# ace19-dev/gvcnn-tf

Hardware: AMD Instinct MI355X
Metric: views/sec (higher is better)
Workload: dtype f32; 1 GPU; BASELINE.json configs[1]: ModelNet-shaped, 12 views x 224x224x3, inception_v3 backbone (raw tap Mixed_6e, final tap Mixed_7c), num_groups=7, f32, forward only; views_per_gpu=384, global_views=384, num_groups=7, num_classes=10, exchange=none, branch_lanes=3, launch=eager

## Files before the change

gvcnn-tf_amd/backbones.py:

```python
import ctypes as C
import os

import numpy as np
import torch

from . import _lib

INCEPTION_BN_EPS = 0.001
RESNET_BN_EPS = 1e-5

INCEPTION_ENDPOINTS = [
    "Conv2d_1a_3x3", "Conv2d_2a_3x3", "Conv2d_2b_3x3", "MaxPool_3a_3x3", "Conv2d_3b_1x1",
    "Conv2d_4a_3x3", "MaxPool_5a_3x3", "Mixed_5b", "Mixed_5c", "Mixed_5d", "Mixed_6a", "Mixed_6b",
    "Mixed_6c", "Mixed_6d", "Mixed_6e", "Mixed_7a", "Mixed_7b", "Mixed_7c"]

SLOT_INPUT, SLOT_WEIGHTS, SLOT_SS, SLOT_ACT0 = 0, 1, 2, 3


def _same_pads(in_size, k, s):
    out = -(-in_size // s)
    total = max((out - 1) * s + k - in_size, 0)
    return out, total // 2


# ... 554 lines not shown
            if kind in ("bias", "bias_sum"):
                for n in name.split("|"):
                    shapes[n] = (c,)
            else:
                for leaf in ("beta", "moving_mean", "moving_variance") + (("gamma",) if has_gamma else ()):
                    shapes[name + "/" + leaf] = (c,)
        return shapes

    def _ptr_table(self, x):
        assert x.is_contiguous() and x.dtype == torch.float32
        assert x.numel() == self.nb * self.height * self.width * 3, (tuple(x.shape), self.nb)
        if self._ptrs is None:
            self._ptrs = (C.c_void_p * len(self._bufs))()
            for i, b in enumerate(self._bufs):
                self._ptrs[i] = b.data_ptr() if b is not None else 0
        self._ptrs[SLOT_INPUT] = x.data_ptr()
        return self._ptrs

    def run(self, x, stream=None):
        ptrs = self._ptr_table(x)
        _lib.check(self.lib.gv_plan_run(self._plan, ptrs, len(self._bufs), _stream_ptr(stream)),
                   "gv_plan_run")

    def run_range(self, x, first, count, stream=None):
        ptrs = self._ptr_table(x)
        _lib.check(self.lib.gv_plan_run_range(self._plan, first, count, ptrs, len(self._bufs),
                                              _stream_ptr(stream)), "gv_plan_run_range")

    def declined_fused_pools(self):
        fused = [i for i, op in enumerate(self.ops) if op["kind"] == "conv" and (op.get("maxpool") or op.get("chain"))]
        if not fused:
            return []
        x = torch.zeros(self.nb * self.height * self.width * 3, dtype=torch.float32, device=self.weights.device)
        declined = []
        for i in fused:
            rc = self.lib.gv_plan_run_range(self._plan, i, 1, self._ptr_table(x), len(self._bufs), _stream_ptr(None))
            if rc == _lib.GV_E_UNSUPPORTED:
                declined.append(self.ops[i]["name"])
            else:
                _lib.check(rc, "gv_plan_run_range(%s)" % self.ops[i]["name"])
        torch.cuda.synchronize(self.weights.device)
        self._ptrs[SLOT_INPUT] = 0
        return declined

    def apply_tiles(self, table):
        for i, op in enumerate(self.ops):
            if op["kind"] == "conv" and op["name"] in table and not op.get("maxpool") and not op.get("chain"):
                op["tile"] = int(table[op["name"]]) + 1
                _lib.check(self.lib.gv_plan_set_conv_tile(self._plan, i, op["tile"]), "gv_plan_set_conv_tile")

    def autotune(self, x, iters=3, verbose=False, in_sequence=4):
        lib = self.lib
        ncfg_plan = lib.gv_conv2d_num_tile_cfgs(self.math_mode if self.dtype == _lib.GV_F32 else -1)
        ncfg_p3 = lib.gv_conv2d_num_tile_cfgs(-3)
        self.run(x)
        chosen, cands = {}, {}
        try:
            for i, op in enumerate(self.ops):
                if op["kind"] != "conv" or op.get("chain"):
                    continue
                ncfg = ncfg_p3 if op["x"].p3 else ncfg_plan
                timed = []
                for t in range(ncfg):
                    lib.gv_conv2d_set_tile_override(t)
                    try:
                        timed.append((self.time_range(x, i, 1, iters), t))
                    except _lib.GvError:
                        continue
                finals = []
                for _, t in sorted(timed)[:3]:
                    lib.gv_conv2d_set_tile_override(t)
                    finals.append((min(self.time_range(x, i, 1, 2 * iters), self.time_range(x, i, 1, 2 * iters)), t))
                best_ms, best = min(finals) if finals else (float("inf"), 0)
                op["tile"] = best + 1
                chosen[op["name"]] = (best, best_ms)
                order = [best] + [t for _, t in sorted(timed) if t != best]
                cands[i] = order[:max(int(in_sequence), 1)]
                _lib.check(lib.gv_plan_set_conv_tile(self._plan, i, best + 1), "gv_plan_set_conv_tile")
                if verbose:
                    print("autotune %-60s cfg %2d  %.4f ms" % (op["name"][-60:], best, best_ms))
        finally:
            lib.gv_conv2d_set_tile_override(-1)
        if int(in_sequence) > 1 and cands:
            seq = {i: {} for i in cands}
            for r in range(int(in_sequence)):
                for i, c in cands.items():
                    _lib.check(lib.gv_plan_set_conv_tile(self._plan, i, c[min(r, len(c) - 1)] + 1), "gv_plan_set_conv_tile")
                each = [min(a, b) for a, b in zip(self.time_each(x, 2 * iters), self.time_each(x, 2 * iters))]
                for i, c in cands.items():
                    t = c[min(r, len(c) - 1)]
                    seq[i][t] = min(each[i], seq[i].get(t, float("inf")))
            moved = 0
            for i, c in cands.items():
                op = self.ops[i]
                best = min(c, key=lambda t: (seq[i][t], c.index(t)))
                moved += best != c[0]
                op["tile"] = best + 1
                chosen[op["name"]] = (best, seq[i][best])
                _lib.check(lib.gv_plan_set_conv_tile(self._plan, i, best + 1), "gv_plan_set_conv_tile")
                if verbose:
                    print("in sequence %-57s cfg %2d  %.4f ms  (warm-repeat choice cfg %2d: %.4f ms in sequence)"
                          % (op["name"][-57:], best, seq[i][best], c[0], seq[i][c[0]]))
            self.autotune_moved = moved
        return chosen

    def time_range(self, x, first, count, iters, stream=None):
# ... 351 lines not shown
```

gvcnn-tf_amd/csrc/conv_bf16s.hip:

```cpp
#include <type_traits>

#include "conv_common.h"
#include "conv_x3_epi.h"

namespace {

using gvconv::ConvArgs;

typedef __bf16 bf16x8 __attribute__((ext_vector_type(8)));
typedef __bf16 bf16x2 __attribute__((ext_vector_type(2)));
typedef unsigned u32x4 __attribute__((ext_vector_type(4)));

constexpr int KT = 16;

__host__ __device__ constexpr int prod_count(int np) { return np == 3 ? 6 : (np == 2 ? 3 : 1); }
__host__ __device__ constexpr int prod_pa(int np, int t) {
    return np == 3 ? (t == 0 ? 2 : (t == 2 || t == 3 ? 1 : 0)) : (np == 2 ? (t == 0 ? 1 : 0) : 0);
}
__host__ __device__ constexpr int prod_pb(int np, int t) {
    return np == 3 ? (t == 1 ? 2 : (t == 2 || t == 4 ? 1 : 0)) : (np == 2 ? (t == 1 ? 1 : 0) : 0);
}

template <int NP>
__device__ __forceinline__ void split8(f32x4 lo, f32x4 hi, bool ok, u32x4 (&out)[NP]) {
// ... 1138 lines not shown
template <int WM, int WN, int TM, int TN, int NP>
int launch_cfg(const ConvArgs& a0, bool generic, hipStream_t st) {
    constexpr int BM = WM * TM * 32, BN = WN * TN * 32;
    ConvArgs a = a0;
    a.tiles_n = gv_ceil_div(a.cout, BN);
    const int tiles_m = gv_ceil_div(a.M, BM);
    const int64_t nwg = (int64_t)tiles_m * a.tiles_n;
    if (nwg > 0x7fffffff) return GV_E_UNSUPPORTED;
    size_t lds = (size_t)(2 * BM + 2 * BN) * (NP * 32 + 16) + (generic ? (size_t)a.Kpad * 8 : 0);
    if (a.y_p3 | a.y2_p3) {
        const size_t epi = (size_t)(WM * WN) * X3EpiGeom<TN>::BYTES;
        lds = lds > epi ? lds : epi;
    }
    if (generic) {
        if (lds > 64 * 1024) {
            const bool ok = GV_BIG_LDS_OK((&conv_igemm_bf16s<WM, WN, TM, TN, NP, true>), 160 * 1024);
            if (!ok) return GV_E_UNSUPPORTED;
        }
        hipLaunchKernelGGL((conv_igemm_bf16s<WM, WN, TM, TN, NP, true>), dim3((unsigned)nwg), dim3(WM * WN * 64), lds, st, a);
    } else {
        if (lds > 64 * 1024) {
            const bool ok = GV_BIG_LDS_OK((&conv_igemm_bf16s<WM, WN, TM, TN, NP, false>), 160 * 1024);
            if (!ok) return GV_E_UNSUPPORTED;
        }
        hipLaunchKernelGGL((conv_igemm_bf16s<WM, WN, TM, TN, NP, false>), dim3((unsigned)nwg), dim3(WM * WN * 64), lds, st, a);
    }
    GV_LAUNCH_CHECK();
    return GV_OK;
}

template <int NP>
int launch_np(int cfg, const ConvArgs& a, bool generic, hipStream_t st) {
    switch (cfg) {
        case 0: return launch_cfg<2, 2, 2, 2, NP>(a, generic, st);
        case 1: return launch_cfg<2, 2, 2, 1, NP>(a, generic, st);
        case 2: return launch_cfg<2, 2, 1, 1, NP>(a, generic, st);
        case 3: return launch_cfg<4, 1, 1, 3, NP>(a, generic, st);
        case 4: return launch_cfg<2, 2, 1, 2, NP>(a, generic, st);
        case 5: return launch_cfg<4, 1, 1, 1, NP>(a, generic, st);
        case 6: return launch_cfg<4, 2, 2, 2, NP>(a, generic, st);
        case 7: return launch_cfg<2, 4, 2, 2, NP>(a, generic, st);
        case 8: return launch_cfg<4, 2, 2, 1, NP>(a, generic, st);
        case 9: return launch_cfg<2, 2, 2, 3, NP>(a, generic, st);
        case 10: return launch_cfg<2, 2, 1, 3, NP>(a, generic, st);
    }
    return GV_E_UNSUPPORTED;
}

}

namespace gvconv {

int bf16s_num_cfgs() { return kNumTiles + 1 + wsg_x3_num_cfgs(); }
int bf16s_special_cfg() { return kNumTiles; }

bool bf16s_stem_ok(int planes, const ConvArgs& a) {
    return planes == 3 && !a.y_p3 && a.cin == 3 && a.kh == a.kw && (a.kw == 3 || a.kw == 7) && a.stride == 2 && a.cout <= 64 &&
           a.dil_shift == 0 && a.split == 0 && a.y2 == nullptr && a.res == nullptr &&
           (int64_t)a.nb * a.ih * a.iw * a.x_ld < 0x7fffffffll;
}

bool bf16s_halo_ok(int planes, const ConvArgs& a, bool generic) {
    return planes == 3 && !generic && !a.y_p3 && a.kh == 3 && a.kw == 3 && a.stride == 1 && a.cin == 32 && a.cout <= 64 &&
           a.dil_shift == 0 && a.split == 0 && a.y2 == nullptr && a.oh == a.ih + 2 * a.pad_t - 2 &&
           a.ow == a.iw + 2 * a.pad_l - 2;
}

bool bf16s_halo_pool_ok(int planes, const ConvArgs& a, bool generic) {
    return a.pool == 1 && bf16s_halo_ok(planes, a, generic) && a.res == nullptr && a.cout % 4 == 0 && a.oh >= 3 && a.ow >= 3 &&
           !(gv_ceil_div(a.ow, 16) * 16 * 5 <= gv_ceil_div(a.ow, 30) * 32 * 4);
}

int bf16s_pick_tile(int , int M, int N, int ) {
    int best = 0;
    double best_cost = 1e30;
    const int order[] = {0, 3, 1, 5};
    const double pen[] = {1.00, 1.02, 1.05, 1.20};
    for (int t = 0; t < 4; ++t) {
        const int bn = kTiles[order[t]].bn;
        const double cost = (double)gv_ceil_div(N, bn) * bn * pen[t];
        if (cost < best_cost) { best_cost = cost; best = order[t]; }
    }
    const int64_t blocks = (int64_t)gv_ceil_div(M, 128) * gv_ceil_div(N, kTiles[best].bn);
    if (blocks < 1024) {
        if (kTiles[best].bn == 128) best = 4;
        else if (kTiles[best].bn == 64) best = 2;
    }
    return best;
}

int bf16s_launch(int planes, int cfg, const ConvArgs& a0, bool generic, hipStream_t st) {
    ConvArgs a = a0;
    a.Kpad = (a.K + KT - 1) / KT * KT;
    a.ktiles = a.Kpad / KT;
    if (cfg == kNumTiles) {
        if (a.pool) return bf16s_halo_pool_ok(planes, a, generic) ? launch_halo_x3(a, st) : GV_E_UNSUPPORTED;
        if (bf16s_stem_ok(planes, a)) return launch_stem_x3(a, st);
        return bf16s_halo_ok(planes, a, generic) ? launch_halo_x3(a, st) : GV_E_UNSUPPORTED;
    }
    if (cfg > kNumTiles) return planes == 3 && !generic ? wsg_x3_launch(cfg - kNumTiles - 1, a0, st) : GV_E_UNSUPPORTED;
    switch (planes) {
        case 3: return launch_np<3>(cfg, a, generic, st);
        case 2: return launch_np<2>(cfg, a, generic, st);
        case 1: return launch_np<1>(cfg, a, generic, st);
    }
    return GV_E_UNSUPPORTED;
// ... 25 lines not shown
```

gvcnn-tf_amd/csrc/conv_common.h:

```cpp
#pragma once
#include "gv_common.h"
#include "conv_stats.h"

namespace gvconv {

struct ConvArgs {
    const float* x;
    const void* w;
    const float* scale;
    const float* shift;
    const float* res;
    float* y;
    float* y2;
    const float* scale2;
    const float* shift2;
    int nb, ih, iw, cin, x_ld;
    int kh, kw, stride, pad_t, pad_l;
    int oh, ow, cout, y_ld, res_ld, y2_ld;
    int M, K, Kpad, ktiles;
    int relu, relu2, split;
    int relu_limit;
    int tiles_n;
    int dil_shift;
#ifdef GV_PHASE_TIMES
// ... 59 lines not shown
                const int m = rbase + (r & 3) + 8 * (r >> 2);
                if (m >= a.M) continue;
                float v = acc[i][j][r] * sc + sh;
                if (a.res) v += a.res[(size_t)m * a.res_ld + col];
                if (dual) {
                    float v2 = v * sc2 + sh2;
                    if (a.relu2) v2 = fmaxf(v2, 0.f);
                    a.y2[(size_t)m * a.y2_ld + col] = v2;
                }
                if (relu) v = fmaxf(v, 0.f);
                ybase[(size_t)m * yld] = v;
            }
        }
    }
}

int bf16s_num_cfgs();
int bf16s_special_cfg();
int bf16s_pick_tile(int planes, int M, int N, int K);
bool bf16s_halo_ok(int planes, const ConvArgs& a, bool generic);
bool bf16s_halo_pool_ok(int planes, const ConvArgs& a, bool generic);
bool bf16s_stem_ok(int planes, const ConvArgs& a);
int bf16s_launch(int planes, int cfg, const ConvArgs& a, bool generic, hipStream_t st);
int bf16s_pack_filter(const float* w_hwio, int kh, int kw, int cin, int cout, int planes, void* out,
                      hipStream_t st);
int64_t bf16s_packed_bytes(int kh, int kw, int cin, int cout, int planes);


int lp_num_cfgs();
int lp_pick_tile(int M, int N, int K);
bool lp_xpre_cfg_ok(int cfg);
int lp_xpre_pick(int M, int N);
bool lp_halo_ok(const ConvArgs& a, bool generic);
bool lp_halo_pool_ok(const ConvArgs& a, bool generic);
bool lp_stem_pool_ok(const ConvArgs& a, bool xf32);
bool lp_stem_ok(const ConvArgs& a, bool xf32);
int lp_launch(int dtype, int cfg, const ConvArgs& a, bool generic, bool xf32, hipStream_t st);
int lp_pack_filter(const float* w_hwio, int kh, int kw, int cin, int cout, int dtype, void* out, hipStream_t st);
int64_t lp_packed_bytes(int kh, int kw, int cin, int cout);
int lp_pack_filters_batched(const gv_pack_job* jobs_dev, const int* block_job_dev, int nblocks, int dtype, hipStream_t st);
int lp_special_cfg();

int dma_lp_num_cfgs();
bool dma_lp_ok(const ConvArgs& a, bool generic, bool xf32);
int dma_lp_launch(int dtype, int cfg, const ConvArgs& a, hipStream_t st);
const void* dma_zero_page();
bool chain_tail_ok(const ConvArgs& a);
int chain_tail_launch(int dtype, const ConvArgs& a, hipStream_t st);
int ws_lp_num_cfgs();
int ws_lp_launch(int dtype, int cfg, const ConvArgs& a, hipStream_t st);
int dma_x3_num_cfgs();
bool dma_x3_ok(const ConvArgs& a);
int dma_x3_launch(int cfg, const ConvArgs& a, hipStream_t st);
int ws_x3_num_cfgs();
int ws_x3_launch(int cfg, const ConvArgs& a, hipStream_t st);
int wsg_x3_num_cfgs();
int wsg_x3_launch(int cfg, const ConvArgs& a, hipStream_t st);

}
```

gvcnn-tf_amd/csrc/conv_igemm.hip:

```cpp
#include "conv_common.h"

namespace {

using gvconv::ConvArgs;

constexpr int CH = 16;
constexpr int KPAD_ALIGN = 32;

template <int WM, int WN, int TM, int TN, int NCH, bool GENERIC>
__global__ __launch_bounds__(256) void conv_igemm_f32(const ConvArgs a) {
    static_assert(WM * WN == 4, "4 waves per workgroup");
    constexpr int BM = WM * TM * 32;
    constexpr int BN = WN * TN * 32;
    constexpr int BKT = CH * NCH;
    constexpr int LDS_LD = BKT + 4;
    constexpr int QPR = BKT / 4;
    constexpr int A_LOADS = (BM * QPR + 255) / 256;
    constexpr int B_LOADS = (BN * QPR + 255) / 256;

    extern __shared__ __attribute__((aligned(16))) float smem[];
    float* sA = smem;
    float* sB = smem + 2 * BM * LDS_LD;

    const int tid = threadIdx.x;
// ... 258 lines not shown
        case 9: return launch_cfg<4, 1, 1, 1, 2>(a, generic, st);
        case 10: return launch_cfg<2, 2, 1, 1, 2>(a, generic, st);
        case 11: return launch_cfg<2, 2, 1, 2, 2>(a, generic, st);
    }
    return GV_E_UNSUPPORTED;
}

int pick_tile(int M, int N, int K) {
    int best = 1;
    double best_cost = 1e30;
    const int order[] = {0, 2, 1, 3};
    const double pen[] = {1.00, 1.00, 1.03, 1.10};
    for (int t = 0; t < 4; ++t) {
        const int bn = kTiles[order[t]].bn;
        const double cost = (double)gv_ceil_div(N, bn) * bn * pen[t];
        if (cost < best_cost) { best_cost = cost; best = order[t]; }
    }
    const int64_t blocks = (int64_t)gv_ceil_div(M, 128) * gv_ceil_div(N, kTiles[best].bn);
    if (blocks < 1024) {
        if (kTiles[best].bn == 128) best = 5;
        else if (kTiles[best].bn == 64) best = 4;
    }
    if (K >= 64) best += 6;
    return best;
}

}

extern "C" void gv_conv2d_set_tile_override(int cfg) { g_tile_override = cfg; }
extern "C" void gv_conv2d_set_debug(int bits) { g_debug = bits; }
#ifdef GV_PHASE_TIMES
unsigned long long* g_phase_buf = nullptr;
extern "C" void gv_conv2d_set_phase_buffer(void* p) { g_phase_buf = (unsigned long long*)p; }
#endif
static int planes_of(int math_mode) {
    switch (math_mode) {
        case GV_MATH_F32: return 0;
        case GV_MATH_BF16X3: return 3;
        case GV_MATH_BF16X2: return 2;
        case GV_MATH_BF16X1: return 1;
    }
    return -1;
}

extern "C" int gv_conv2d_special_tile_cfg(int32_t math_mode) {
    if (math_mode == -1) return gvconv::lp_special_cfg();
    const int np = planes_of(math_mode);
    return np <= 0 ? GV_E_BADARG : gvconv::bf16s_special_cfg();
}

extern "C" int gv_conv2d_num_tile_cfgs(int32_t math_mode) {
    if (math_mode == -1) return gvconv::lp_num_cfgs();
    if (math_mode == -3) return gvconv::dma_x3_num_cfgs();
    const int np = planes_of(math_mode);
    return np < 0 ? GV_E_BADARG : (np == 0 ? kNumTiles : gvconv::bf16s_num_cfgs());
}

extern "C" int64_t gv_packed_filter_bytes(int32_t kh, int32_t kw, int32_t cin, int32_t cout,
                                          int32_t dtype, int32_t math_mode) {
    if (kh <= 0 || kw <= 0 || cin <= 0 || cout <= 0) return GV_E_BADARG;
    if (dtype == GV_BF16 || dtype == GV_F16) return gvconv::lp_packed_bytes(kh, kw, cin, cout);
    if (dtype != GV_F32) return GV_E_UNSUPPORTED;
    const int np = planes_of(math_mode);
    if (np < 0) return GV_E_BADARG;
    if (np > 0) return gvconv::bf16s_packed_bytes(kh, kw, cin, cout, np);
    const int64_t K = (int64_t)kh * kw * cin;
    return 4 * (int64_t)cout * ((K + KPAD_ALIGN - 1) / KPAD_ALIGN * KPAD_ALIGN);
}

extern "C" int gv_pack_filter_hwio(const float* w_hwio, int32_t kh, int32_t kw, int32_t cin,
                                   int32_t cout, void* w_packed, int32_t dtype, int32_t math_mode,
                                   void* stream) {
    if (!w_hwio || !w_packed || kh <= 0 || kw <= 0 || cin <= 0 || cout <= 0) return GV_E_BADARG;
    if (dtype == GV_BF16 || dtype == GV_F16)
        return gvconv::lp_pack_filter(w_hwio, kh, kw, cin, cout, dtype, w_packed, (hipStream_t)stream);
    if (dtype != GV_F32) return GV_E_UNSUPPORTED;
    const int np = planes_of(math_mode);
    if (np < 0) return GV_E_BADARG;
    if (np > 0) return gvconv::bf16s_pack_filter(w_hwio, kh, kw, cin, cout, np, w_packed, (hipStream_t)stream);
    const int K = kh * kw * cin;
    const int Kpad = (K + KPAD_ALIGN - 1) / KPAD_ALIGN * KPAD_ALIGN;
    const int64_t total = (int64_t)cout * Kpad;
    hipLaunchKernelGGL(pack_filter_hwio_f32, dim3((unsigned)gv_ceil_div(total, 256)), dim3(256), 0,
                       (hipStream_t)stream, w_hwio, K, Kpad, cout, (float*)w_packed);
    GV_LAUNCH_CHECK();
    return GV_OK;
}

extern "C" int gv_pack_filters_batched(const gv_pack_job* jobs_dev, int32_t num_jobs, const int32_t* block_job_dev,
                                       int32_t num_blocks, int32_t dtype, void* stream) {
    if (!jobs_dev || !block_job_dev || num_jobs <= 0 || num_blocks <= 0) return GV_E_BADARG;
    if (dtype != GV_BF16 && dtype != GV_F16) return GV_E_UNSUPPORTED;
    return gvconv::lp_pack_filters_batched(jobs_dev, block_job_dev, num_blocks, dtype, (hipStream_t)stream);
}

static int conv2d_fwd_impl(const gv_conv_desc* d, const void* x, const float* xscale, const float* xshift,
                           const void* w_packed, const float* scale, const float* shift, const void* residual,
                           void* y, void* y2, const float* scale2, const float* shift2, void* stream,
                           const gv_bn_stats* stats = nullptr);

extern "C" int gv_conv2d_fwd(const gv_conv_desc* d, const void* x, const void* w_packed,
                             const float* scale, const float* shift, const void* residual,
                             void* y, void* y2, const float* scale2, const float* shift2,
                             void* stream) {
    return conv2d_fwd_impl(d, x, nullptr, nullptr, w_packed, scale, shift, residual, y, y2, scale2, shift2, stream);
}
// ... 4 lines not shown
                                  const float* shift2, void* stream) {
    if (!xscale || !xshift) return GV_E_BADARG;
    return conv2d_fwd_impl(d, x, xscale, xshift, w_packed, scale, shift, residual, y, y2, scale2, shift2, stream);
}

extern "C" int gv_conv2d_fwd_bnstats(const gv_conv_desc* d, const void* x, const void* w_packed, const float* scale,
                                     const float* shift, const void* residual, void* y, const gv_bn_stats* stats,
                                     void* stream) {
    if (!stats) return GV_E_BADARG;
    return conv2d_fwd_impl(d, x, nullptr, nullptr, w_packed, scale, shift, residual, y, nullptr, nullptr, nullptr, stream, stats);
}

static int conv2d_fwd_impl(const gv_conv_desc* d, const void* x, const float* xscale, const float* xshift,
                           const void* w_packed, const float* scale, const float* shift, const void* residual,
                           void* y, void* y2, const float* scale2, const float* shift2, void* stream,
                           const gv_bn_stats* stats) {
    if (!d || !x || !w_packed || !scale || !shift || !y) return GV_E_BADARG;
    if (d->nb <= 0 || d->ih <= 0 || d->iw <= 0 || d->cin <= 0 || d->cout <= 0 || d->kh <= 0 ||
        d->kw <= 0 || d->stride <= 0 || d->oh <= 0 || d->ow <= 0 || d->pad_t < 0 || d->pad_l < 0)
        return GV_E_BADARG;
    const bool split = (d->flags & GV_CONV_SPLIT) != 0;
    if (split) {
        if (!y2 || d->split_col <= 0 || d->split_col >= d->cout) return GV_E_BADARG;
        if (d->y_ld < d->split_col || d->y2_ld < d->cout - d->split_col) return GV_E_BADARG;
    } else {
        if (d->y_ld < d->cout) return GV_E_BADARG;
        if (y2 && (!scale2 || !shift2 || d->y2_ld < d->cout)) return GV_E_BADARG;
    }
    if (d->x_ld < d->cin) return GV_E_BADARG;
    if (residual && d->res_ld < d->cout) return GV_E_BADARG;
    {
        if (d->in_dilation != 2 && d->y_step != 2 && ((d->oh - 1) * d->stride - d->pad_t >= d->ih ||
                                    (d->ow - 1) * d->stride - d->pad_l >= d->iw))
            return GV_E_BADARG;
    }
    const bool lp = d->dtype == GV_BF16 || d->dtype == GV_F16;
    if (d->dtype != GV_F32 && !lp) return GV_E_UNSUPPORTED;
    if ((d->flags & GV_CONV_X_F32) && !lp) return GV_E_BADARG;
    const int np = lp ? 1 : planes_of(d->math_mode);
    if (np < 0) return GV_E_BADARG;
    const bool xp3 = (d->flags & GV_CONV_X_P3) != 0;
    const bool yp3 = (d->flags & GV_CONV_Y_P3) != 0, y2p3 = (d->flags & GV_CONV_Y2_P3) != 0;
    if ((xp3 || yp3 || y2p3) && (lp || np != 3)) return GV_E_BADARG;
    if (y2p3 && !split) return GV_E_BADARG;
    if (yp3 || y2p3) {
        if (d->cout % 8 != 0 || (y2 && !split) || (residual && d->res_ld % 4 != 0)) return GV_E_UNSUPPORTED;
        if (yp3 && (d->y_ld % 16 != 0 || (split ? d->split_col : d->cout) % 16 != 0)) return GV_E_UNSUPPORTED;
        if (y2p3 && (d->y2_ld % 16 != 0 || (d->cout - d->split_col) % 16 != 0 || d->split_col % 8 != 0)) return GV_E_UNSUPPORTED;
        if (!yp3 && (d->y_ld % 4 != 0 || !gv_aligned16(y))) return GV_E_ALIGN;
        if (split && !y2p3 && (d->y2_ld % 4 != 0 || !gv_aligned16(y2))) return GV_E_ALIGN;
        if (split && d->split_col % 8 != 0) return GV_E_UNSUPPORTED;
    }
    const int ncfg = lp ? gvconv::lp_num_cfgs()
                        : (xp3 ? gvconv::dma_x3_num_cfgs() : (np == 0 ? kNumTiles : gvconv::bf16s_num_cfgs()));
    if (d->tile_cfg < 0 || d->tile_cfg > ncfg) return GV_E_BADARG;
    const int64_t M64 = (int64_t)d->nb * d->oh * d->ow;
    if (M64 > 0x7fffffff || (int64_t)d->nb * d->ih * d->iw > 0x7fffffff) return GV_E_UNSUPPORTED;
    if (!gv_aligned16(w_packed)) return GV_E_ALIGN;

    ConvArgs a;
    a.x = (const float*)x; a.w = w_packed; a.scale = scale; a.shift = shift;
    a.res = (const float*)residual; a.y = (float*)y; a.y2 = (float*)y2;
    a.scale2 = scale2; a.shift2 = shift2;
    a.xscale = xscale; a.xshift = xshift;
    a.nb = d->nb; a.ih = d->ih; a.iw = d->iw; a.cin = d->cin; a.x_ld = d->x_ld;
    a.kh = d->kh; a.kw = d->kw; a.stride = d->stride; a.pad_t = d->pad_t; a.pad_l = d->pad_l;
    a.oh = d->oh; a.ow = d->ow; a.cout = d->cout; a.y_ld = d->y_ld; a.res_ld = d->res_ld;
    a.y2_ld = d->y2_ld;
    a.M = (int)M64; a.K = d->kh * d->kw * d->cin;
    a.Kpad = (a.K + KPAD_ALIGN - 1) / KPAD_ALIGN * KPAD_ALIGN;
    a.ktiles = 0;
    a.relu = (d->flags & GV_CONV_RELU) ? 1 : 0;
    a.relu2 = (d->flags & GV_CONV_RELU2) ? 1 : 0;
    a.split = split ? d->split_col : 0;
    if (d->relu_cols < 0) return GV_E_BADARG;
    a.relu_limit = d->relu_cols > 0 ? d->relu_cols : 0x7fffffff;
    a.tiles_n = 0;
    a.dbg = g_debug;
#ifdef GV_PHASE_TIMES
    a.phase_buf = g_phase_buf;
#endif
    a.zeros = nullptr;
    a.y_p3 = (d->flags & GV_CONV_Y_P3) ? 1 : 0;
    a.y2_p3 = (d->flags & GV_CONV_Y2_P3) ? 1 : 0;
    if (d->in_dilation != 0 && d->in_dilation != 1 && d->in_dilation != 2) return GV_E_BADARG;
    a.dil_shift = d->in_dilation == 2 ? 1 : 0;
    if (a.dil_shift && (np == 0 || (d->cin % CH != 0) || d->stride != 1)) return GV_E_UNSUPPORTED;
    if (d->y_step != 0) {
        if (d->y_step != 2 || d->y_py < 0 || d->y_py > 1 || d->y_px < 0 || d->y_px > 1) return GV_E_BADARG;
        if (2 * (d->oh - 1) + d->y_py >= d->y_ih || 2 * (d->ow - 1) + d->y_px >= d->y_iw) return GV_E_BADARG;
        if (!lp || split || y2 || d->stride != 1 || a.dil_shift) return GV_E_UNSUPPORTED;
        if ((int64_t)d->nb * d->y_ih * d->y_iw > 0x7fffffff) return GV_E_UNSUPPORTED;
        a.y_step = 2; a.y_py = d->y_py; a.y_px = d->y_px; a.y_ih = d->y_ih; a.y_iw = d->y_iw;
    }
    a.y_div_img = gv_fast_div(d->oh * d->ow);
    a.y_div_row = gv_fast_div(d->ow);
    if (stats) {
        if (stats->mode != GV_BN_STATS_FWD && stats->mode != GV_BN_STATS_BWD) return GV_E_BADARG;
        if (stats->groups <= 0 || stats->nseg <= 0 || stats->nseg > GV_BN_STATS_MAX_SEG) return GV_E_BADARG;
        if (!lp || split || y2 || (d->flags & (GV_CONV_RELU | GV_CONV_RELU2))) return GV_E_UNSUPPORTED;
        if (d->cout % 8 != 0 || d->y_ld % 8 != 0 || !gv_aligned16(y) || (residual && (d->res_ld % 8 != 0 || !gv_aligned16(residual))))
            return GV_E_UNSUPPORTED;
        a.st.mode = stats->mode == GV_BN_STATS_FWD ? gvconv::STAT_FWD : gvconv::STAT_BWD;
        a.st.hw = d->oh * d->ow;
        a.st.G = stats->groups;
        a.st.nseg = stats->nseg;
        a.st.hw_magic = a.st.hw > 1 ? (unsigned)((0x100000000ull + (unsigned)a.st.hw - 1) / (unsigned)a.st.hw) : 0u;
// ... 111 lines not shown
```

gvcnn-tf_amd/csrc/conv_ws_x3.hip:

```cpp
#include <cstdlib>
#include <type_traits>

#include "conv_common.h"
#include "conv_lp_epi.h"
#include "conv_x3_epi.h"

namespace {

constexpr int X3W_HEAD = 64;
constexpr int X3W_NL = 4;

struct WsX3Args {
    int taps, nchunks, nk;
    int halo_lo;
    int strip_blocks;
    int pad_[3];
};

__device__ __forceinline__ void x3w_dma16(const char* gsrc, char* lds_dst) {
    __builtin_amdgcn_global_load_lds((const __attribute__((address_space(1))) void*)gsrc,
                                     (__attribute__((address_space(3))) void*)lds_dst, 16, 0, 0);
}
template <int N>
__device__ __forceinline__ void x3w_wait_vm() {
    static_assert(N >= 0 && N < 64, "vmcnt is a 6-bit counter");
    asm volatile("s_waitcnt vmcnt(%0)" ::"n"(N) : "memory");
}

__device__ __forceinline__ void x3w_gload16(f32x4& dst, const char* p) {
    asm volatile("global_load_dwordx4 %0, %1, off" : "=v"(dst) : "v"(p) : "memory");
}
template <int N>
__device__ __forceinline__ void x3w_wait_vm_reg(f32x4& r) {
    static_assert(N >= 0 && N < 64, "vmcnt is a 6-bit counter");
    asm volatile("s_waitcnt vmcnt(%1)" : "+v"(r) : "n"(N) : "memory");
}

template <int WM, int WN, int TM, int TN, int NB, int SBMAX, int GEMM = 0>
__global__ __launch_bounds__((WM * WN + X3W_NL) * 64, 3) void conv_ws_x3(const ConvArgs a, const WsX3Args w) {
    constexpr int NC = WM * WN;
    constexpr int BM = WM * TM * 32, BN = WN * TN * 32;
    constexpr int B_PLANE = BN * 32, B_SLOT = 3 * B_PLANE;
    constexpr int A_PLANE = GEMM ? BM * 32 : X3W_HEAD + SBMAX * 1024, S_BUF = 3 * A_PLANE;
    constexpr int NA = GEMM ? 3 : 2;
    constexpr int OFF_S = NB * B_SLOT;
    constexpr int UB3 = 3 * (BN / 32);
    constexpr int LB = (UB3 + X3W_NL - 1) / X3W_NL;
    static_assert(NC == 8, "eight consumer waves + four loaders: three waves per SIMD");
    static_assert(TM <= TN && TM * TN >= 4, "plane-2 fragments of a and b share one register block");
    static_assert(NB >= 3 && (NB - 1) * LB < 64, "ring depth / vmcnt range");
    static_assert(GEMM == 0 || (NB == 4 && BM % (16 * X3W_NL) == 0), "GEMM mode: four filter slots, 16-row load instructions");
    (void)NA;

    extern __shared__ __attribute__((aligned(128))) char smem[];
    const int tid = threadIdx.x;
    const int lane = tid & 63;
    const int wave = __builtin_amdgcn_readfirstlane(tid >> 6);
    const int lid = gv_xcd_remap(blockIdx.x, gridDim.x);
    const int tile_n = lid % a.tiles_n, tile_m = lid / a.tiles_n;
    const int m0 = tile_m * BM, n0 = tile_n * BN;
    const int nk = w.nk, NTAP = w.taps;
    const bool nosync = (a.dbg & (16384 | 65536)) != 0;

    static_assert(BN <= X3W_NL * 64, "one loader thread per tile column");
    float ss_v[2] = {0.f, 0.f};
    f32x16 acc[TM][TN];

    if (wave >= NC) {
        const int lw = wave - NC;
        if (tid - NC * 64 < BN) {
            const int cc = min(n0 + tid - NC * 64, a.cout - 1);
            ss_v[0] = a.scale[cc];
            ss_v[1] = a.shift[cc];
        }
        if (!(a.dbg & 16384)) {
            __builtin_amdgcn_s_setprio(3);
            const bool nodma = (a.dbg & 32768) != 0, nobar = (a.dbg & 65536) != 0;
            const int lrow = lane >> 1;
            const int lc16 = (((lane & 1) ^ ((lrow >> 3) & 1)) << 4);
            const char* xb = reinterpret_cast<const char*>(a.x);
            const char* b_ptr[LB];
            int b_dst[LB];
            {
                const size_t wrow = (size_t)(a.Kpad / 16) * 96;
#pragma unroll
                for (int i = 0; i < LB; ++i) {
                    int d = lw + i * X3W_NL;
                    d = d < UB3 ? d : UB3 - 1;
                    const int rb = d / 3, p = d - rb * 3;
                    int n = n0 + rb * 32 + lrow;
                    n = n < a.cout ? n : a.cout - 1;
                    b_ptr[i] = reinterpret_cast<const char*>(a.w) + (size_t)n * wrow + p * 32 + lc16;
                    b_dst[i] = p * B_PLANE + rb * 1024;
                }
            }
            int bq_t = 0, bq_c = 0, bq_slot = 0;
            const int gtap = (a.cin >> 4) * 96;
            auto issue_b = [&]() {
                const unsigned koff = (unsigned)(bq_t * gtap + bq_c * 96);
                char* sb = smem + bq_slot * B_SLOT;
#pragma unroll
                for (int i = 0; i < LB; ++i)
                    if (!nodma) x3w_dma16(b_ptr[i] + koff, sb + b_dst[i]);
                if (++bq_t == NTAP) { bq_t = 0; ++bq_c; }
                bq_slot = bq_slot + 1 == NB ? 0 : bq_slot + 1;
            };
            if constexpr (GEMM != 0) {
                constexpr int RPW = BM / X3W_NL, NI = RPW / 16;
                const int qd = lane & 3;
                const char* a_ptr[NI];
                int a_dst[NI];
#pragma unroll
                for (int i = 0; i < NI; ++i) {
                    const int row = lw * RPW + i * 16 + (lane >> 2);
                    int m = m0 + row;
                    m = m < a.M ? m : a.M - 1;
                    a_ptr[i] = xb + (size_t)(unsigned)m * ((size_t)a.x_ld * 4) + qd * 16;
                    a_dst[i] = OFF_S + row * 32 + ((((qd >> 1) ^ ((row >> 3) & 1))) << 4) + (qd & 1) * 8;
                }
                f32x4 stg[2][NI];
                auto load_a = [&](auto sc, int c) {
                    constexpr int S = decltype(sc)::value;
                    c = c < nk ? c : nk - 1;
#pragma unroll
                    for (int i = 0; i < NI; ++i) x3w_gload16(stg[S][i], a_ptr[i] + (size_t)c * 64);
                };
                auto wait_a = [&](auto sc, auto nc) {
                    constexpr int S = decltype(sc)::value;
                    constexpr int N = decltype(nc)::value;
#pragma unroll
                    for (int i = 0; i < NI; ++i) x3w_wait_vm_reg<N>(stg[S][i]);
                };
                auto write_a = [&](auto sc, int slot) {
                    constexpr int S = decltype(sc)::value;
                    char* sb = smem + slot * S_BUF;
#pragma unroll
                    for (int i = 0; i < NI; ++i) {
                        float v[4] = {stg[S][i][0], stg[S][i][1], stg[S][i][2], stg[S][i][3]};
#pragma unroll
                        for (int p = 0; p < 3; ++p) {
                            const unsigned lo = pack2<__bf16>(v[0], v[1]), hi = pack2<__bf16>(v[2], v[3]);
                            typedef unsigned u32x2_t __attribute__((ext_vector_type(2)));
                            *reinterpret_cast<u32x2_t*>(sb + p * A_PLANE + a_dst[i]) = u32x2_t{lo, hi};
                            if (p < 2) {
                                v[0] -= __builtin_bit_cast(float, lo << 16);
                                v[1] -= __builtin_bit_cast(float, lo & 0xffff0000u);
                                v[2] -= __builtin_bit_cast(float, hi << 16);
                                v[3] -= __builtin_bit_cast(float, hi & 0xffff0000u);
                            }
                        }
                    }
                };
                using S0 = std::integral_constant<int, 0>;
                using S1 = std::integral_constant<int, 1>;
                auto fetch = [&](auto sc, int k) {
                    issue_b();
                    load_a(sc, k);
                };
                fetch(S0{}, 0);
                fetch(S1{}, 1);
                wait_a(S0{}, std::integral_constant<int, 0>{});
                wait_a(S1{}, std::integral_constant<int, 0>{});
                write_a(S0{}, 0);
                write_a(S1{}, 1);
                fetch(S0{}, 2);
                fetch(S1{}, 3);
                asm volatile("s_waitcnt lgkmcnt(0)" ::: "memory");
                if (!nobar) __builtin_amdgcn_s_barrier();
                auto iter = [&](auto sc, int j) {
                    wait_a(sc, std::integral_constant<int, LB + NI>{});
                    if (j + 2 < nk) {
                        int slot = j + 2;
                        slot -= (slot / 3) * 3;
                        write_a(sc, slot);
                        asm volatile("s_waitcnt lgkmcnt(0)" ::: "memory");
                    }
                    if (!nobar) __builtin_amdgcn_s_barrier();
                    if (j + 4 >= nk) {
                        bq_c = nk - 1;
                        bq_slot = (nk - 1) & 3;
                    }
                    fetch(sc, j + 4);
                };
                for (int j = 0; j + 1 < nk; j += 2) {
                    iter(S0{}, j);
                    if (j + 2 < nk) iter(S1{}, j + 1);
                }
                x3w_wait_vm<0>();
            } else {
            const unsigned pix_bytes = (unsigned)a.x_ld * 6u;
            int sq_c = 0, sq_buf = 0;
            int sp_blk = 1 << 30, sp_p = 0, sp_c = 0, sp_buf = 0;
            auto strip_begin = [&]() {
                sp_blk = lw / 3; sp_p = lw - sp_blk * 3; sp_c = sq_c; sp_buf = sq_buf;
                ++sq_c;
                sq_buf ^= 1;
            };
            auto strip_units = [&](int n) {
                char* sb = smem + OFF_S + sp_buf * S_BUF + X3W_HEAD;
                const unsigned coff = (unsigned)sp_c * 96u + (unsigned)lc16;
                for (int i = 0; i < n && sp_blk < w.strip_blocks; ++i) {
                    int p = m0 - w.halo_lo + sp_blk * 32 + lrow;
                    p = p < 0 ? 0 : (p < a.M ? p : a.M - 1);
                    if (!nodma) x3w_dma16(xb + (size_t)(unsigned)p * pix_bytes + coff + sp_p * 32, sb + sp_p * A_PLANE + sp_blk * 1024);
                    ++sp_p; ++sp_blk;
                    if (sp_p == 3) { sp_p = 0; ++sp_blk; }
                }
            };
            const int upl = (3 * w.strip_blocks + X3W_NL - 1) / X3W_NL;
            const int win = max(NTAP - NB + 2, 1);
            const int ppi = (upl + win - 1) / win;
            strip_begin();
            strip_units(1 << 20);
            issue_b();
#pragma unroll
            for (int q = 1; q < NB; ++q) issue_b();
            x3w_wait_vm<(NB - 2) * LB>();
            if (!nobar) __builtin_amdgcn_s_barrier();
            if (w.nchunks > 1) { strip_begin(); strip_units(ppi); }
            int ft = 0;
            for (int j = 0; j + 1 < nk; ++j) {
                if (j + NB - 1 <= nk - 1) x3w_wait_vm<(NB - 3) * LB>();
                else x3w_wait_vm<0>();
                if (!nobar) __builtin_amdgcn_s_barrier();
                const bool last_tap = ft + 1 == NTAP;
                if (last_tap && sq_c < w.nchunks) strip_begin();
                strip_units(ppi);
                if (j + NB < nk) issue_b();
                ft = last_tap ? 0 : ft + 1;
            }
            x3w_wait_vm<0>();
            }
        }
    } else {
        const int wm = wave / WN, wn = wave % WN;
        const int r = lane & 31, h = lane >> 5;
        if constexpr (GEMM == 0) {
            if (tid < 96) {
                const int img = tid >> 4;
// ... 102 lines not shown
                    if (j == TN - 1) { A1[i] = lds16(aa[i] + A_PLANE); X3W_PIN(); }
                    if (i == TM - 1) { B1[j] = lds16(bn + j * 1024 + B_PLANE); X3W_PIN(); }
                }
            }
            X3W_PIN();
        };
        int q_fr = 0, q_fs = 0, q_tap = 0;
        int sbuf = 0, bslot = 0;
        int aa[TM];
#pragma unroll
        for (int i = 0; i < TM; ++i) aa[i] = a_addr(i, -(a.pad_t * a.iw + a.pad_l), 0, OFF_S);
        asm volatile("s_waitcnt lgkmcnt(0)" ::: "memory");
        if (!nosync) __builtin_amdgcn_s_barrier();
#pragma unroll
        for (int i = 0; i < TM; ++i) { A0[i] = lds16(aa[i]); A1[i] = lds16(aa[i] + A_PLANE); }
#pragma unroll
        for (int j = 0; j < TN; ++j) {
            B0[j] = lds16(b_lane + j * 1024);
            B1[j] = lds16(b_lane + j * 1024 + B_PLANE);
            T[j] = lds16(b_lane + j * 1024 + 2 * B_PLANE);
        }
        int bn = 0;
        auto next_addr = [&]() {
            if constexpr (GEMM != 0) {
                sbuf = sbuf + 1 == NA ? 0 : sbuf + 1;
#pragma unroll
                for (int i = 0; i < TM; ++i) aa[i] = a_addr(i, 0, 0, OFF_S + sbuf * S_BUF);
                bslot = bslot + B_SLOT == NB * B_SLOT ? 0 : bslot + B_SLOT;
                bn = b_lane + bslot;
                return;
            }
            const bool wrap = q_tap + 1 == NTAP;
            const bool row_end = q_fs + 1 == a.kw;
            q_tap = wrap ? 0 : q_tap + 1;
            q_fr = wrap ? 0 : (row_end ? q_fr + 1 : q_fr);
            q_fs = (wrap || row_end) ? 0 : q_fs + 1;
            sbuf = wrap ? sbuf ^ 1 : sbuf;
            const int sbase = OFF_S + sbuf * S_BUF;
            const int off = (q_fr - a.pad_t) * a.iw + (q_fs - a.pad_l);
#pragma unroll
            for (int i = 0; i < TM; ++i) aa[i] = a_addr(i, off, q_tap, sbase);
            bslot = bslot + B_SLOT == NB * B_SLOT ? 0 : bslot + B_SLOT;
            bn = b_lane + bslot;
        };
        for (int j = 0; j + 1 < nk; ++j) {
            kstep(std::true_type{}, aa, bn, !nosync, next_addr);
        }
        kstep(std::false_type{}, aa, bn, false, [] {});
#undef X3W_PIN
    }
    __syncthreads();
    constexpr int SS_OFF = NC * X3EpiGeom<TN>::BYTES;
    float* sstab = reinterpret_cast<float*>(smem + SS_OFF);
    if (tid >= NC * 64 && tid - NC * 64 < BN) {
        sstab[tid - NC * 64] = ss_v[0];
        sstab[BN + tid - NC * 64] = ss_v[1];
    }
    __syncthreads();
    if (wave < NC) {
        const int wm = wave / WN, wn = wave % WN;
        x3_epilogue_staged<TM, TN>(a, acc, m0, n0, wm, wn, lane, reinterpret_cast<float*>(smem + wave * X3EpiGeom<TN>::BYTES), sstab, BN);
    }
}

#ifndef GV_KERNEL_ONLY
bool ws_x3_epi_ok(const ConvArgs& a) {
    if (a.cout % 8 != 0 || (a.y2 != nullptr && a.split == 0)) return false;
    if (a.res != nullptr && (a.res_ld % 4 != 0 || !gv_aligned16(a.res))) return false;
    if (!a.y_p3 && (a.y_ld % 4 != 0 || !gv_aligned16(a.y))) return false;
    if (a.split > 0 && (a.split % 8 != 0 || (!a.y2_p3 && (a.y2_ld % 4 != 0 || !gv_aligned16(a.y2))))) return false;
    return true;
}

bool ws_x3_shape_ok(const ConvArgs& a) {
    return a.stride == 1 && a.dil_shift == 0 && a.oh == a.ih && a.ow == a.iw && a.cin % 16 == 0 && a.x_ld % 16 == 0 &&
           a.kh * a.kw <= 32 && a.kw < 32 && a.pad_t < a.kh && a.pad_l < a.kw && a.pool == 0 && a.xscale == nullptr &&
           a.y_step == 0 && a.st.mode == gvconv::STAT_OFF && ws_x3_epi_ok(a);
}

template <int WM, int WN, int TM, int TN, int NB, int SBMAX>
int launch_ws_x3(const ConvArgs& a0, hipStream_t st) {
    constexpr int NC = WM * WN, BM = WM * TM * 32, BN = WN * TN * 32;
    if (!ws_x3_shape_ok(a0)) return GV_E_UNSUPPORTED;
    ConvArgs a = a0;
    a.Kpad = a.K;
    WsX3Args w;
    w.taps = a.kh * a.kw;
    w.nchunks = a.cin / 16;
    w.nk = w.taps * w.nchunks;
    if (w.nk < NB || w.taps < NB - 1) return GV_E_UNSUPPORTED;
    w.halo_lo = a.pad_t * a.iw + a.pad_l;
    const int halo_hi = (a.kh - 1 - a.pad_t) * a.iw + (a.kw - 1 - a.pad_l);
    w.strip_blocks = gv_ceil_div(w.halo_lo + BM + halo_hi, 32);
    if (w.strip_blocks > SBMAX) return GV_E_UNSUPPORTED;
    w.pad_[0] = w.pad_[1] = w.pad_[2] = 0;
    a.tiles_n = gv_ceil_div(a.cout, BN);
    const int64_t nwg = (int64_t)gv_ceil_div(a.M, BM) * a.tiles_n;
    if (nwg > 0x7fffffff) return GV_E_UNSUPPORTED;
    constexpr size_t ring = (size_t)NB * 96 * BN + 6 * (size_t)(X3W_HEAD + SBMAX * 1024);
    constexpr size_t epi = (size_t)NC * X3EpiGeom<TN>::BYTES + 2 * BN * sizeof(float);
    constexpr size_t lds = ring > epi ? ring : epi;
    static_assert(lds <= 160 * 1024, "one workgroup per CU");
    auto kern = &conv_ws_x3<WM, WN, TM, TN, NB, SBMAX, 0>;
    if (lds > 64 * 1024) {
        const bool ok = GV_BIG_LDS_OK(kern, 160 * 1024);
        if (!ok) return GV_E_UNSUPPORTED;
    }
    hipLaunchKernelGGL(kern, dim3((unsigned)nwg), dim3((NC + X3W_NL) * 64), lds, st, a, w);
    GV_LAUNCH_CHECK();
    return GV_OK;
}

template <int WM, int WN, int TM, int TN, int MODE>
int launch_wsg_x3(const ConvArgs& a0, hipStream_t st) {
    constexpr int NC = WM * WN, BM = WM * TM * 32, BN = WN * TN * 32, NB = 4;
    const ConvArgs& c = a0;
    if (!(c.kh == 1 && c.kw == 1 && c.stride == 1 && c.pad_t == 0 && c.pad_l == 0 && c.dil_shift == 0 && c.oh == c.ih &&
          c.ow == c.iw && c.cin % 16 == 0 && c.x_ld % 4 == 0 && gv_aligned16(c.x) && c.pool == 0 && c.xscale == nullptr &&
          c.y_step == 0 && c.st.mode == gvconv::STAT_OFF && ws_x3_epi_ok(c)))
        return GV_E_UNSUPPORTED;
    ConvArgs a = a0;
    a.Kpad = a.K;
    WsX3Args w;
    w.taps = 1;
    w.nchunks = a.cin / 16;
    w.nk = w.nchunks;
    if (w.nk < 4) return GV_E_UNSUPPORTED;
    w.halo_lo = 0;
    w.strip_blocks = 0;
    w.pad_[0] = w.pad_[1] = w.pad_[2] = 0;
    a.tiles_n = gv_ceil_div(a.cout, BN);
    const int64_t nwg = (int64_t)gv_ceil_div(a.M, BM) * a.tiles_n;
    if (nwg > 0x7fffffff) return GV_E_UNSUPPORTED;
    constexpr size_t ring = (size_t)NB * 96 * BN + 9 * (size_t)BM * 32;
    constexpr size_t epi = (size_t)NC * X3EpiGeom<TN>::BYTES + 2 * BN * sizeof(float);
    constexpr size_t lds = ring > epi ? ring : epi;
    static_assert(lds <= 160 * 1024, "one workgroup per CU");
    auto kern = &conv_ws_x3<WM, WN, TM, TN, NB, 0, MODE>;
    if (lds > 64 * 1024) {
        const bool ok = GV_BIG_LDS_OK(kern, 160 * 1024);
        if (!ok) return GV_E_UNSUPPORTED;
    }
    hipLaunchKernelGGL(kern, dim3((unsigned)nwg), dim3((NC + X3W_NL) * 64), lds, st, a, w);
    GV_LAUNCH_CHECK();
    return GV_OK;
}
#endif

}

#ifndef GV_KERNEL_ONLY
namespace gvconv {

int ws_x3_num_cfgs() { return 5; }

int ws_x3_launch(int cfg, const ConvArgs& a, hipStream_t st) {
    static const bool off = getenv("GV_NO_WS") != nullptr;
    if (off) return GV_E_UNSUPPORTED;
    switch (cfg) {
        case 0: return launch_ws_x3<4, 2, 2, 3, 4, 13>(a, st);
        case 1: return launch_ws_x3<4, 2, 2, 2, 4, 13>(a, st);
        case 2: return launch_ws_x3<8, 1, 2, 3, 3, 21>(a, st);
        case 3: return launch_ws_x3<8, 1, 2, 2, 3, 21>(a, st);
        case 4: return launch_ws_x3<8, 1, 1, 5, 4, 13>(a, st);
    }
    return GV_E_UNSUPPORTED;
}

int wsg_x3_num_cfgs() { return 2; }

int wsg_x3_launch(int cfg, const ConvArgs& a, hipStream_t st) {
    static const bool off = getenv("GV_NO_WS") != nullptr;
    if (off) return GV_E_UNSUPPORTED;
    switch (cfg) {
        case 0: return launch_wsg_x3<4, 2, 2, 3, 1>(a, st);
        case 1: return launch_wsg_x3<4, 2, 2, 2, 1>(a, st);
    }
    return GV_E_UNSUPPORTED;
}

}
#endif
```

Before: 30070 views/s.

## Add deeper-pipelined and light-tile warp-specialized bf16x3 GEMM configs to autotune

Generalizes the warp-specialized bf16x3 1x1-conv GEMM kernel over the number of filter ring slots, the count of register stages used for A loads, and the number of loader waves. It then exposes three more tile configurations to the autotuner in bf16x3 math mode: a wide-N tile with four A register stages, a wide-N tile with four ring slots, and a light 4+2-wave tile meant to fit two workgroups per CU. The aim is to hide global-load latency better and to raise occupancy on small 1x1 convolutions. The price is more autotune time, more kernel instantiations and more register pressure, and the reworked vmcnt wait counts carry a correctness risk.

```diff
diff --git a/gvcnn-tf_amd/backbones.py b/gvcnn-tf_amd/backbones.py
--- a/gvcnn-tf_amd/backbones.py
+++ b/gvcnn-tf_amd/backbones.py
@@ -630,6 +630,8 @@
     def autotune(self, x, iters=3, verbose=False, in_sequence=4):
         lib = self.lib
         ncfg_plan = lib.gv_conv2d_num_tile_cfgs(self.math_mode if self.dtype == _lib.GV_F32 else -1)
+        if self.dtype == _lib.GV_F32 and self.math_mode == _lib.GV_MATH_BF16X3:
+            ncfg_plan = lib.gv_conv2d_num_tile_cfgs(-4)
         ncfg_p3 = lib.gv_conv2d_num_tile_cfgs(-3)
         self.run(x)
         chosen, cands = {}, {}
diff --git a/gvcnn-tf_amd/csrc/conv_bf16s.hip b/gvcnn-tf_amd/csrc/conv_bf16s.hip
--- a/gvcnn-tf_amd/csrc/conv_bf16s.hip
+++ b/gvcnn-tf_amd/csrc/conv_bf16s.hip
@@ -1214,6 +1214,7 @@
 namespace gvconv {
 
 int bf16s_num_cfgs() { return kNumTiles + 1 + wsg_x3_num_cfgs(); }
+int bf16s_num_ext_cfgs() { return kNumTiles + 1 + wsg_x3_num_ext_cfgs(); }
 int bf16s_special_cfg() { return kNumTiles; }
 
 bool bf16s_stem_ok(int planes, const ConvArgs& a) {
diff --git a/gvcnn-tf_amd/csrc/conv_common.h b/gvcnn-tf_amd/csrc/conv_common.h
--- a/gvcnn-tf_amd/csrc/conv_common.h
+++ b/gvcnn-tf_amd/csrc/conv_common.h
@@ -135,9 +135,11 @@
 int dma_x3_num_cfgs();
 bool dma_x3_ok(const ConvArgs& a);
 int dma_x3_launch(int cfg, const ConvArgs& a, hipStream_t st);
+int bf16s_num_ext_cfgs();
 int ws_x3_num_cfgs();
 int ws_x3_launch(int cfg, const ConvArgs& a, hipStream_t st);
 int wsg_x3_num_cfgs();
+int wsg_x3_num_ext_cfgs();
 int wsg_x3_launch(int cfg, const ConvArgs& a, hipStream_t st);
 
 }
diff --git a/gvcnn-tf_amd/csrc/conv_igemm.hip b/gvcnn-tf_amd/csrc/conv_igemm.hip
--- a/gvcnn-tf_amd/csrc/conv_igemm.hip
+++ b/gvcnn-tf_amd/csrc/conv_igemm.hip
@@ -334,6 +334,7 @@
 extern "C" int gv_conv2d_num_tile_cfgs(int32_t math_mode) {
     if (math_mode == -1) return gvconv::lp_num_cfgs();
     if (math_mode == -3) return gvconv::dma_x3_num_cfgs();
+    if (math_mode == -4) return gvconv::bf16s_num_ext_cfgs();
     const int np = planes_of(math_mode);
     return np < 0 ? GV_E_BADARG : (np == 0 ? kNumTiles : gvconv::bf16s_num_cfgs());
 }
@@ -444,7 +445,8 @@
         if (split && d->split_col % 8 != 0) return GV_E_UNSUPPORTED;
     }
     const int ncfg = lp ? gvconv::lp_num_cfgs()
-                        : (xp3 ? gvconv::dma_x3_num_cfgs() : (np == 0 ? kNumTiles : gvconv::bf16s_num_cfgs()));
+                        : (xp3 ? gvconv::dma_x3_num_cfgs()
+                               : (np == 0 ? kNumTiles : (np == 3 ? gvconv::bf16s_num_ext_cfgs() : gvconv::bf16s_num_cfgs())));
     if (d->tile_cfg < 0 || d->tile_cfg > ncfg) return GV_E_BADARG;
     const int64_t M64 = (int64_t)d->nb * d->oh * d->ow;
     if (M64 > 0x7fffffff || (int64_t)d->nb * d->ih * d->iw > 0x7fffffff) return GV_E_UNSUPPORTED;
diff --git a/gvcnn-tf_amd/csrc/conv_ws_x3.hip b/gvcnn-tf_amd/csrc/conv_ws_x3.hip
--- a/gvcnn-tf_amd/csrc/conv_ws_x3.hip
+++ b/gvcnn-tf_amd/csrc/conv_ws_x3.hip
@@ -36,8 +36,8 @@
     asm volatile("s_waitcnt vmcnt(%1)" : "+v"(r) : "n"(N) : "memory");
 }
 
-template <int WM, int WN, int TM, int TN, int NB, int SBMAX, int GEMM = 0>
-__global__ __launch_bounds__((WM * WN + X3W_NL) * 64, 3) void conv_ws_x3(const ConvArgs a, const WsX3Args w) {
+template <int WM, int WN, int TM, int TN, int NB, int SBMAX, int GEMM = 0, int AD = 2, int NL = X3W_NL>
+__global__ __launch_bounds__((WM * WN + NL) * 64, 3) void conv_ws_x3(const ConvArgs a, const WsX3Args w) {
     constexpr int NC = WM * WN;
     constexpr int BM = WM * TM * 32, BN = WN * TN * 32;
     constexpr int B_PLANE = BN * 32, B_SLOT = 3 * B_PLANE;
@@ -45,11 +45,13 @@
     constexpr int NA = GEMM ? 3 : 2;
     constexpr int OFF_S = NB * B_SLOT;
     constexpr int UB3 = 3 * (BN / 32);
-    constexpr int LB = (UB3 + X3W_NL - 1) / X3W_NL;
-    static_assert(NC == 8, "eight consumer waves + four loaders: three waves per SIMD");
+    constexpr int LB = (UB3 + NL - 1) / NL;
+    static_assert(NC == 2 * NL && (NL == 4 || (NL == 2 && GEMM != 0)),
+                  "eight consumer waves + four loaders: three waves per SIMD (GEMM mode's light tile: 4 + 2, two workgroups per CU)");
     static_assert(TM <= TN && TM * TN >= 4, "plane-2 fragments of a and b share one register block");
     static_assert(NB >= 3 && (NB - 1) * LB < 64, "ring depth / vmcnt range");
-    static_assert(GEMM == 0 || (NB == 4 && BM % (16 * X3W_NL) == 0), "GEMM mode: four filter slots, 16-row load instructions");
+    static_assert(GEMM == 0 || ((NB == 3 || NB == 4) && BM % (16 * NL) == 0), "GEMM mode: three or four filter slots, 16-row load instructions");
+    static_assert(AD == 2 || AD == 4, "register stages of the GEMM mode's A loads");
     (void)NA;
 
     extern __shared__ __attribute__((aligned(128))) char smem[];
@@ -62,16 +64,22 @@
     const int nk = w.nk, NTAP = w.taps;
     const bool nosync = (a.dbg & (16384 | 65536)) != 0;
 
-    static_assert(BN <= X3W_NL * 64, "one loader thread per tile column");
-    float ss_v[2] = {0.f, 0.f};
+    constexpr int CPT = (BN + NL * 64 - 1) / (NL * 64);
+    float ss_v[2 * CPT];
+#pragma unroll
+    for (int q = 0; q < 2 * CPT; ++q) ss_v[q] = 0.f;
     f32x16 acc[TM][TN];
 
     if (wave >= NC) {
         const int lw = wave - NC;
-        if (tid - NC * 64 < BN) {
-            const int cc = min(n0 + tid - NC * 64, a.cout - 1);
-            ss_v[0] = a.scale[cc];
-            ss_v[1] = a.shift[cc];
+#pragma unroll
+        for (int q = 0; q < CPT; ++q) {
+            const int c = tid - NC * 64 + q * NL * 64;
+            if (c < BN) {
+                const int cc = min(n0 + c, a.cout - 1);
+                ss_v[2 * q] = a.scale[cc];
+                ss_v[2 * q + 1] = a.shift[cc];
+            }
         }
         if (!(a.dbg & 16384)) {
             __builtin_amdgcn_s_setprio(3);
@@ -85,7 +93,7 @@
                 const size_t wrow = (size_t)(a.Kpad / 16) * 96;
 #pragma unroll
                 for (int i = 0; i < LB; ++i) {
-                    int d = lw + i * X3W_NL;
+                    int d = lw + i * NL;
                     d = d < UB3 ? d : UB3 - 1;
                     const int rb = d / 3, p = d - rb * 3;
                     int n = n0 + rb * 32 + lrow;
@@ -106,7 +114,7 @@
                 bq_slot = bq_slot + 1 == NB ? 0 : bq_slot + 1;
             };
             if constexpr (GEMM != 0) {
-                constexpr int RPW = BM / X3W_NL, NI = RPW / 16;
+                constexpr int RPW = BM / NL, NI = RPW / 16;
                 const int qd = lane & 3;
                 const char* a_ptr[NI];
                 int a_dst[NI];
@@ -118,7 +126,7 @@
                     a_ptr[i] = xb + (size_t)(unsigned)m * ((size_t)a.x_ld * 4) + qd * 16;
                     a_dst[i] = OFF_S + row * 32 + ((((qd >> 1) ^ ((row >> 3) & 1))) << 4) + (qd & 1) * 8;
                 }
-                f32x4 stg[2][NI];
+                f32x4 stg[AD][NI];
                 auto load_a = [&](auto sc, int c) {
                     constexpr int S = decltype(sc)::value;
                     c = c < nk ? c : nk - 1;
@@ -153,22 +161,33 @@
                 };
                 using S0 = std::integral_constant<int, 0>;
                 using S1 = std::integral_constant<int, 1>;
+                using SA = std::integral_constant<int, 2 % AD>;
+                using SB = std::integral_constant<int, 3 % AD>;
+                constexpr int OPS = LB + NI;
+                constexpr int NW_A = (AD - 1) * OPS, NW_B = (NB - 3) * OPS + NI;
+                constexpr int NW = NW_A < NW_B ? NW_A : NW_B;
                 auto fetch = [&](auto sc, int k) {
                     issue_b();
                     load_a(sc, k);
                 };
                 fetch(S0{}, 0);
                 fetch(S1{}, 1);
-                wait_a(S0{}, std::integral_constant<int, 0>{});
-                wait_a(S1{}, std::integral_constant<int, 0>{});
+                if constexpr (AD == 4) {
+                    load_a(std::integral_constant<int, 2>{}, 2);
+                    load_a(std::integral_constant<int, 3>{}, 3);
+                }
+                wait_a(S0{}, std::integral_constant<int, (AD - 2) * NI>{});
+                wait_a(S1{}, std::integral_constant<int, (AD - 2) * NI>{});
                 write_a(S0{}, 0);
                 write_a(S1{}, 1);
-                fetch(S0{}, 2);
-                fetch(S1{}, 3);
+                if constexpr (NB == 4) issue_b();
+                load_a(S0{}, AD);
+                fetch(S1{}, AD + 1);
                 asm volatile("s_waitcnt lgkmcnt(0)" ::: "memory");
                 if (!nobar) __builtin_amdgcn_s_barrier();
                 auto iter = [&](auto sc, int j) {
-                    wait_a(sc, std::integral_constant<int, LB + NI>{});
+                    if (nodma) x3w_wait_vm<0>();
+                    wait_a(sc, std::integral_constant<int, NW>{});
                     if (j + 2 < nk) {
                         int slot = j + 2;
                         slot -= (slot / 3) * 3;
@@ -176,15 +195,19 @@
                         asm volatile("s_waitcnt lgkmcnt(0)" ::: "memory");
                     }
                     if (!nobar) __builtin_amdgcn_s_barrier();
-                    if (j + 4 >= nk) {
+                    if (j + NB >= nk) {
                         bq_c = nk - 1;
-                        bq_slot = (nk - 1) & 3;
+                        bq_slot = (nk - 1) % NB;
                     }
-                    fetch(sc, j + 4);
+                    fetch(sc, j + 2 + AD);
                 };
-                for (int j = 0; j + 1 < nk; j += 2) {
-                    iter(S0{}, j);
-                    if (j + 2 < nk) iter(S1{}, j + 1);
+                for (int j = 0; j + 1 < nk; j += AD) {
+                    iter(SA{}, j);
+                    if (j + 2 < nk) iter(SB{}, j + 1);
+                    if constexpr (AD == 4) {
+                        if (j + 3 < nk) iter(S0{}, j + 2);
+                        if (j + 4 < nk) iter(S1{}, j + 3);
+                    }
                 }
                 x3w_wait_vm<0>();
             } else {
@@ -393,9 +416,15 @@
     __syncthreads();
     constexpr int SS_OFF = NC * X3EpiGeom<TN>::BYTES;
     float* sstab = reinterpret_cast<float*>(smem + SS_OFF);
-    if (tid >= NC * 64 && tid - NC * 64 < BN) {
-        sstab[tid - NC * 64] = ss_v[0];
-        sstab[BN + tid - NC * 64] = ss_v[1];
+    if (tid >= NC * 64) {
+#pragma unroll
+        for (int q = 0; q < CPT; ++q) {
+            const int c = tid - NC * 64 + q * NL * 64;
+            if (c < BN) {
+                sstab[c] = ss_v[2 * q];
+                sstab[BN + c] = ss_v[2 * q + 1];
+            }
+        }
     }
     __syncthreads();
     if (wave < NC) {
@@ -452,9 +481,9 @@
     return GV_OK;
 }
 
-template <int WM, int WN, int TM, int TN, int MODE>
+template <int WM, int WN, int TM, int TN, int MODE, int NB = 4, int AD = 2, int NL = X3W_NL>
 int launch_wsg_x3(const ConvArgs& a0, hipStream_t st) {
-    constexpr int NC = WM * WN, BM = WM * TM * 32, BN = WN * TN * 32, NB = 4;
+    constexpr int NC = WM * WN, BM = WM * TM * 32, BN = WN * TN * 32;
     const ConvArgs& c = a0;
     if (!(c.kh == 1 && c.kw == 1 && c.stride == 1 && c.pad_t == 0 && c.pad_l == 0 && c.dil_shift == 0 && c.oh == c.ih &&
           c.ow == c.iw && c.cin % 16 == 0 && c.x_ld % 4 == 0 && gv_aligned16(c.x) && c.pool == 0 && c.xscale == nullptr &&
@@ -476,13 +505,13 @@
     constexpr size_t ring = (size_t)NB * 96 * BN + 9 * (size_t)BM * 32;
     constexpr size_t epi = (size_t)NC * X3EpiGeom<TN>::BYTES + 2 * BN * sizeof(float);
     constexpr size_t lds = ring > epi ? ring : epi;
-    static_assert(lds <= 160 * 1024, "one workgroup per CU");
-    auto kern = &conv_ws_x3<WM, WN, TM, TN, NB, 0, MODE>;
+    static_assert(lds <= (NL == 2 ? 80 : 160) * 1024, "one workgroup per CU (the light tile: two)");
+    auto kern = &conv_ws_x3<WM, WN, TM, TN, NB, 0, MODE, AD, NL>;
     if (lds > 64 * 1024) {
         const bool ok = GV_BIG_LDS_OK(kern, 160 * 1024);
         if (!ok) return GV_E_UNSUPPORTED;
     }
-    hipLaunchKernelGGL(kern, dim3((unsigned)nwg), dim3((NC + X3W_NL) * 64), lds, st, a, w);
+    hipLaunchKernelGGL(kern, dim3((unsigned)nwg), dim3((NC + NL) * 64), lds, st, a, w);
     GV_LAUNCH_CHECK();
     return GV_OK;
 }
@@ -509,6 +538,7 @@
 }
 
 int wsg_x3_num_cfgs() { return 2; }
+int wsg_x3_num_ext_cfgs() { return 5; }
 
 int wsg_x3_launch(int cfg, const ConvArgs& a, hipStream_t st) {
     static const bool off = getenv("GV_NO_WS") != nullptr;
@@ -516,6 +546,9 @@
     switch (cfg) {
         case 0: return launch_wsg_x3<4, 2, 2, 3, 1>(a, st);
         case 1: return launch_wsg_x3<4, 2, 2, 2, 1>(a, st);
+        case 2: return launch_wsg_x3<2, 4, 2, 3, 1, 3, 4>(a, st);
+        case 4: return launch_wsg_x3<2, 2, 2, 2, 1, 3, 2, 2>(a, st);
+        case 3: return launch_wsg_x3<2, 4, 2, 2, 1, 4, 2>(a, st);
     }
     return GV_E_UNSUPPORTED;
 }
```

After: 30180 views/s, median of 2. No clear change (+0.4%).
